# SJLeo/GCC

Measured on AMD Instinct MI355X. Metric: training images/sec at 256x256 (pix2pix GCC), higher is better.
Workload: dtype bf16

## Files before the change

gcc_amd/csrc/conv_igemm.hip:

```cpp
#include <stdlib.h>
#include <mutex>
#include "common.hpp"
#include "igemm_common.hpp"

#ifndef GCC_IGEMM_ROT
#define GCC_IGEMM_ROT 0
#endif

namespace gcc_igemm {

#ifdef GCC_CLOCK_PROBE
__device__ unsigned long long g_clock_probe[4096][8];
#endif

template <int BP, int BC, bool UT, int NS = 2, bool EV = false>
__global__ __launch_bounds__((BP / 32) * 64) void igemm_kernel(const IgemmArgs<EV> p) {
    constexpr int EPI = EV ? 1 : 0;
#include "igemm_kernel_body.inc"
}

template <int BP, int BC, bool UT, int NS = 2>
__global__ __launch_bounds__((BP / 32) * 64) void igemm_ex_kernel(const IgemmExParams p) {
    constexpr int EPI = 2;
#include "igemm_kernel_body.inc"
// ... 795 lines not shown
    auto stage_row = [&](int y) {
        char* base = ylds + ((y + 1) % 3) * row_bytes;
        const bool row_ok = (unsigned)y < (unsigned)a.Ho;
        for (int q = wave; q < pieces; q += NW) {
            const int o = q * 1024 + lane * 16;
            const int pp = o / THIN_WIDE_RB, slot = (o % THIN_WIDE_RB) >> 4;
            const int co = ((slot ^ (pp & 15)) << 3);
            const int ox = pp - 2;
            const bool ok = row_ok && (unsigned)ox < (unsigned)a.Wo && co < a.Co8;
            const uint32_t off = ok ? (uint32_t)((((n * a.Ho + y) * a.Wo + ox) * a.ldy + a.yoff + co) * 2) : OOB;
            __builtin_amdgcn_raw_ptr_buffer_load_lds(rs_y, LDS_PTR(void, base + q * 1024), 16, off, 0, 0, 0);
        }
    };
    stage_row(r_first);
    stage_row(r_first + 1);
    for (int f2 = wave; f2 < 2 * NK; f2 += NW) {
        const int py = f2 / NK, f = f2 - py * NK;
        const int u = f / (3 * NCC), b = (f / NCC) % 3 - 1, cc = f % NCC;
        const int px = i >> 3, ci = i & 7;
        const int kh = py == 0 ? (u == 0 ? 1 : 3) : (u == 0 ? 0 : 2);
        const int kw = px == 0 ? (b == 0 ? 1 : (b < 0 ? 3 : -1)) : (b > 0 ? 0 : (b == 0 ? 2 : -1));
        const int co = 32 * cc + 8 * g;
        const uint32_t off = (kw >= 0 && ci < a.Ci && co < a.Co8) ? (uint32_t)((((ci * 16 + kh * 4 + kw) * a.Co8) + co) * 2) : OOB;
        *(i32x4*)(wlds + (f2 * 64 + lane) * 16) = __builtin_amdgcn_raw_buffer_load_b128(rs_w, off, 0, 0);
    }
    int yoffs[3][NCC];
#pragma unroll
    for (int bb = 0; bb < 3; bb++)
#pragma unroll
        for (int cc = 0; cc < NCC; cc++) {
            const int pp = i + (bb - 1) + 2;
            yoffs[bb][cc] = pp * THIN_WIDE_RB + (((4 * cc + g) ^ (pp & 15)) << 4);
        }
    const int ci0 = (g & 1) * 4, pxo = g >> 1;
    float bv[4];
#pragma unroll
    for (int e = 0; e < 4; e++) bv[e] = (a.bias && ci0 + e < a.Ci) ? a.bias[ci0 + e] : 0.f;
    asm volatile("s_waitcnt vmcnt(0)" ::: "memory");
    __syncthreads();
#pragma unroll 1
    for (int r = r_first; r <= r_last; r++) {
        if (r < r_last) stage_row(r + 2);
        const char* row_u0 = ylds + ((r + 2) % 3) * row_bytes;
        const char* row_u1 = ylds + ((r + 1) % 3) * row_bytes;
#pragma unroll
        for (int pass = 0; pass < 2; pass++) {
            const int py = pass == 0 ? 1 : 0;
            const int iy = pass == 0 ? 2 * r + 1 : 2 * r + 2;
            if ((unsigned)iy >= (unsigned)a.H) continue;
            const char* wp = wlds + (py * NK * 64 + lane) * 16;
            for (int jt = wave; jt < a.tiles_per_row; jt += NW) {
                const char* t0 = row_u0 + jt * (16 * THIN_WIDE_RB);
                const char* t1 = row_u1 + jt * (16 * THIN_WIDE_RB);
                f32x4 acc0 = {0.f, 0.f, 0.f, 0.f}, acc1 = {0.f, 0.f, 0.f, 0.f};
                constexpr int PF = 4;
                bf16x8 yv[NK], wv[NK];
                auto rdy = [&](int ff) {
                    const int u = ff / (3 * NCC), bb = (ff / NCC) % 3, cc = ff % NCC;
                    return *(const bf16x8*)((u == 0 ? t0 : t1) + yoffs[bb][cc]);
                };
#pragma unroll
                for (int f = 0; f < PF; f++) { yv[f] = rdy(f); wv[f] = *(const bf16x8*)(wp + f * 1024); }
                __builtin_amdgcn_sched_group_barrier(0x100, 2 * PF, 0);
#pragma unroll
                for (int f = 0; f < NK; f++) {
                    if (f + PF < NK) { yv[f + PF] = rdy(f + PF); wv[f + PF] = *(const bf16x8*)(wp + (f + PF) * 1024); }
                    if (f & 1) acc1 = __builtin_amdgcn_mfma_f32_16x16x32_bf16(wv[f], yv[f], acc1, 0, 0, 0);
                    else acc0 = __builtin_amdgcn_mfma_f32_16x16x32_bf16(wv[f], yv[f], acc0, 0, 0, 0);
                    __builtin_amdgcn_sched_group_barrier(0x008, 1, 0);
                    if (f + PF < NK) __builtin_amdgcn_sched_group_barrier(0x100, 2, 0);
                }
                const int ix = 2 * (jt * 16 + i) + pxo;
                if (ix < a.W) {
                    float o[4];
#pragma unroll
                    for (int e = 0; e < 4; e++) {
                        o[e] = apply_act(acc0[e] + acc1[e] + bv[e], a.act, a.slope);
                        if (ci0 + e >= a.Ci) o[e] = 0.f;
                    }
                    i32x2 v = {(int)pack2bf(o[0], o[1]), (int)pack2bf(o[2], o[3])};
                    *(i32x2*)(a.dx + ((size_t)(n * a.H + iy) * a.W + ix) * a.ldx + a.xoff + ci0) = v;
                }
            }
        }
        asm volatile("s_waitcnt vmcnt(0)" ::: "memory");
        __syncthreads();
    }
}

static bool thin_dgrad_wide_shape(const gcc_conv_t* c) {
    return ceil8(c->Ci) == 8 && c->KH == 4 && c->KW == 4 && c->stride == 2 && c->pad == 1 && !(c->H & 1) && !(c->W & 1) &&
           c->Co > 64 && c->Co <= 128 && ((c->W / 2) & 3) == 0 && (size_t)(c->W / 2 + 4) * THIN_WIDE_RB * 3 + 48 * 1024 <= 156 * 1024 &&
           gcc_opt(GCC_OPT_IGEMM_THIN) >= 1 && gcc_opt(GCC_OPT_IGEMM_THIN) != 2;
}
static bool thin_dgrad_shape(const gcc_conv_t* c) {
    if (thin_dgrad_wide_shape(c)) return true;
    return ceil8(c->Ci) == 8 && c->KH == 4 && c->KW == 4 && c->stride == 2 && c->pad == 1 && !(c->H & 1) && !(c->W & 1) &&
           c->Co >= 16 && c->Co <= 64 && thin_enabled();
}
static int launch_thin_dgrad(const gcc_conv_t* c, const void* dy, const void* wt, void* dx, const gcc_epilogue_t* ep, hipStream_t st) {
    ThinDgradArgs a;
    a.dy = (const bf16_t*)dy; a.wt = (const bf16_t*)wt; a.dx = (bf16_t*)dx;
    a.bias = ep ? ep->bias : nullptr; a.act = ep ? ep->act : GCC_ACT_NONE; a.slope = ep ? ep->slope : 0.f;
    a.N = c->N; a.H = c->H; a.W = c->W; a.Ho = c->H / 2; a.Wo = c->W / 2;
    a.ldy = c->ldy; a.yoff = c->yoff; a.ldx = c->ldx; a.xoff = c->xoff; a.Ci = c->Ci; a.Co8 = ceil8(c->Co);
    const size_t yb = (size_t)c->N * a.Ho * a.Wo * c->ldy * 2, wb = (size_t)c->Ci * 16 * a.Co8 * 2;
    const size_t xb = (size_t)c->N * c->H * c->W * c->ldx * 2;
    if (yb >= OOB || wb >= OOB || xb >= OOB) return -1;
    a.dy_bytes = (uint32_t)yb; a.wt_bytes = (uint32_t)wb;
    a.tiles_per_row = cdiv(a.Wo, 16);
    a.ntiles = c->N * a.Ho * a.tiles_per_row;
    a.dTpr = make_fastdiv(a.tiles_per_row); a.dHh = make_fastdiv(a.Ho);
    if (thin_dgrad_wide_shape(c)) {
        const size_t lds = (size_t)3 * (a.Wo + 4) * THIN_WIDE_RB + 48 * 1024;
        static std::once_flag wide_once;
        std::call_once(wide_once, [] {
            (void)hipFuncSetAttribute((const void*)thin_dgrad_wide_kernel, hipFuncAttributeMaxDynamicSharedMemorySize, 156 * 1024);
        });
        int wpi = 256 / c->N;
        if (wpi < 1) wpi = 1;
        if (wpi > a.Ho) wpi = a.Ho;
        const int rows_per_wg = cdiv(a.Ho, wpi);
        wpi = cdiv(a.Ho, rows_per_wg);
        hipLaunchKernelGGL(thin_dgrad_wide_kernel, dim3(c->N * wpi), dim3(THIN_WIDE_NT), lds, st, a, rows_per_wg, wpi);
        GCC_CHECK_LAUNCH();
        return GCC_OK;
    }
    const int ncc = a.Co8 > 32 ? 2 : 1;
    int wgs = cdiv(a.ntiles, 4);
    if (wgs > 768) wgs = 768;
    const dim3 grid(wgs, 2);
    if (ncc == 2) hipLaunchKernelGGL(thin_dgrad_k4s2_kernel<2>, grid, dim3(256), 0, st, a);
    else hipLaunchKernelGGL(thin_dgrad_k4s2_kernel<1>, grid, dim3(256), 0, st, a);
    GCC_CHECK_LAUNCH();
    return GCC_OK;
}

extern "C" int gcc_conv_y2_supported(const gcc_conv_t* c, int dgrad, const gcc_epilogue_t* ep) {
    if (check_conv(c) || dgrad || !ep || !thin_shape(c)) return 0;
    if (ep->stats_partial || ep->act == GCC_ACT_TANH || (ep->act == GCC_ACT_LRELU && (ep->slope < 0.f || ep->slope > 1.f))) return 0;
    if ((ep->ldy2 & 7) || (ep->y2off & 7)) return 0;
    if (ep->y2_mode == 1) return ep->act == GCC_ACT_LRELU || ep->act == GCC_ACT_NONE;
    if (ep->y2_mode == 2) return ep->y2_gate != nullptr;
    return 0;
}

int gcc_internal_thinout_fprop(const gcc_conv_t* c, const void* x, const void* w, void* y, const gcc_epilogue_t* ep, hipStream_t st);
int gcc_internal_thinout_dgrad(const gcc_conv_t* c, const void* dy, const void* wt, void* dx, const gcc_epilogue_t* ep, hipStream_t st);
int gcc_internal_ring3(const gcc_conv_t* c, int dgrad, const void* src, const void* w, void* dst, const gcc_epilogue_t* ep, hipStream_t st);
int gcc_internal_ring3_rows(const gcc_conv_t* c, int dgrad);
bool gcc_internal_ring3_routed(const gcc_conv_t* c, int dgrad, const gcc_epilogue_t* ep);

constexpr size_t FUSE_BN_PARTIAL_BYTES = (size_t)4096 * 1024;

int gcc_internal_igemm(const gcc_conv_t* c, int dgrad, const void* src, const void* w, void* dst, const gcc_epilogue_t* ep,
                       int batch, long src_bstride, long wgt_bstride, long dst_bstride, hipStream_t st) {
    GCC_ENTER();
    int rc = check_conv(c);
    if (rc) return rc;
    if (!src || !w || !dst) return GCC_ERR_BAD_ARG;
    const int Ho = gcc_conv_out(c->H, c->KH, c->stride, c->pad);
    const int Wo = gcc_conv_out(c->W, c->KW, c->stride, c->pad);
    if (batch == 1 && head_shape(c) && ep && ep->workspace && !ep->stats_partial && (((uintptr_t)ep->workspace) & 15) == 0) {
        const int taps = c->KH * c->KW;
        if (!dgrad) {
            int ks = 1;
            const size_t need = head_fprop_workspace(c, &ks);
            if (need <= ep->workspace_bytes) {
                IgemmParams q;
                q.src = (const bf16_t*)src; q.wgt = (const bf16_t*)w; q.dst = (bf16_t*)dst; q.bias = nullptr; q.stats = nullptr;
                q.act = GCC_ACT_NONE; q.slope = 0.f;
                q.N = c->N; q.KH = 1; q.KW = 1; q.stride = 1; q.pad = 0; q.dgrad = 0;
                q.Hs = c->H; q.Ws = c->W; q.lds_ = c->ldx; q.soff = c->xoff; q.Hd = c->H; q.Wd = c->W; q.ldd = c->ldy; q.doff = c->yoff;
                q.Ct = ceil8(c->Ci); q.Cout = taps; q.ldw = q.Ct;
                const size_t rows = head_rows(c);
                const size_t sb = rows * (size_t)q.lds_ * 2, wb = (size_t)taps * q.ldw * 2;
                if (sb < OOB && wb < OOB) {
                    q.src_bytes = (uint32_t)sb; q.wgt_bytes = (uint32_t)wb;
                    q.src_bstride = q.wgt_bstride = q.dst_bstride = 0;
                    q.ntiles = 1; q.mtiles_max = cdiv((int)rows, 128);
                    const int nk = cdiv(q.Ct, BK);
                    q.ksplit = ks; q.kper = cdiv(nk, ks); q.partial = (float*)ep->workspace; q.rows_max = (int)rows; q.Cpad = 16;
                    q.raw_partial = 1;
                    int rc2 = launch<128, 16>(q, 1, 1, st);
                    if (rc2) return rc2;
                    HeadArgs a = {};
                    a.partial = q.partial; a.ksplit = q.ksplit; a.rows_max = q.rows_max; a.Cpad = 16;
                    a.bias = ep->bias; a.act = ep->act; a.slope = ep->slope;
                    a.dst = (bf16_t*)dst; a.ldd = c->ldy; a.doff = c->yoff;
                    a.N = c->N; a.H = c->H; a.W = c->W; a.Ho = Ho; a.Wo = Wo; a.KH = c->KH; a.KW = c->KW; a.stride = c->stride; a.pad = c->pad;
                    const size_t outs = (size_t)c->N * Ho * Wo;
                    hipLaunchKernelGGL(head_tapsum_kernel, dim3((unsigned)(outs + 15 > 16 * 4096 ? 4096 : (outs + 15) / 16)), dim3(256), 0, st, a);
                    GCC_CHECK_LAUNCH();
                    return GCC_OK;
                }
            }
        }
    }
    if (batch == 1 && dgrad && thin_dgrad_shape(c) && !(ep && ep->stats_partial)) {
        const int rc2 = launch_thin_dgrad(c, src, w, dst, ep, st);
        if (rc2 >= 0) return rc2;
    }
    if (batch == 1) {
        const int rc3 = dgrad ? gcc_internal_thinout_dgrad(c, src, w, dst, ep, st) : gcc_internal_thinout_fprop(c, src, w, dst, ep, st);
        if (rc3 != GCC_ERR_UNSUPPORTED) return rc3;
        const int rc4 = gcc_internal_ring3(c, dgrad, src, w, dst, ep, st);
        if (rc4 != GCC_ERR_UNSUPPORTED) return rc4;
    }
    if (ep && ep->y2) {
        if (!gcc_conv_y2_supported(c, dgrad, ep)) return GCC_ERR_UNSUPPORTED;
    }
    if (batch == 1 && !dgrad && thin_shape(c) &&
        !(ep && (ep->stats_partial || ep->act == GCC_ACT_TANH || (ep->act == GCC_ACT_LRELU && (ep->slope < 0.f || ep->slope > 1.f))))) {
        const int rc2 = launch_thin(c, src, w, dst, ep, st);
        if (rc2 >= 0) return rc2;
    }
    if (ep && ep->y2) return GCC_ERR_UNSUPPORTED;
    IgemmParams p;
    p.src = (const bf16_t*)src; p.wgt = (const bf16_t*)w; p.dst = (bf16_t*)dst;
    p.bias = ep ? ep->bias : nullptr;
    p.stats = ep ? ep->stats_partial : nullptr;
    p.act = ep ? ep->act : GCC_ACT_NONE;
    p.slope = ep ? ep->slope : 0.f;
    p.N = c->N; p.KH = c->KH; p.KW = c->KW; p.stride = c->stride; p.pad = c->pad; p.dgrad = dgrad;
    size_t src_pix, max_rows;
    if (!dgrad) {
        p.Hs = c->H; p.Ws = c->W; p.lds_ = c->ldx; p.soff = c->xoff;
        p.Hd = Ho; p.Wd = Wo; p.ldd = c->ldy; p.doff = c->yoff;
        p.Ct = ceil8(c->Ci); p.Cout = c->Co;
        max_rows = (size_t)c->N * Ho * Wo;
    } else {
        p.Hs = Ho; p.Ws = Wo; p.lds_ = c->ldy; p.soff = c->yoff;
        p.Hd = c->H; p.Wd = c->W; p.ldd = c->ldx; p.doff = c->xoff;
        p.Ct = ceil8(c->Co); p.Cout = c->Ci;
        const int s = c->stride;
        max_rows = (size_t)c->N * cdiv(c->H, s) * cdiv(c->W, s);
    }
    src_pix = (size_t)p.N * p.Hs * p.Ws;
    p.ldw = c->KH * c->KW * p.Ct;
    const size_t sb = src_pix * (size_t)p.lds_ * 2, wb = (size_t)p.Cout * p.ldw * 2;
    const size_t db = (size_t)p.N * p.Hd * p.Wd * p.ldd * 2;
    if (sb >= OOB || wb >= OOB || db >= (size_t)1 << 32) return GCC_ERR_UNSUPPORTED;
    p.src_bytes = (uint32_t)sb; p.wgt_bytes = (uint32_t)wb;
    p.src_bstride = src_bstride; p.wgt_bstride = wgt_bstride; p.dst_bstride = dst_bstride;
    if (batch < 1 || (batch > 1 && p.stats)) return GCC_ERR_BAD_ARG;
    const int phases = dgrad ? c->stride * c->stride : 1;
    if (dgrad && (c->KH < c->stride || c->KW < c->stride)) return GCC_ERR_UNSUPPORTED;
    const TilePlan tp = select_tile(c->plan, max_rows, p.Cout, phases, conv_nk(c, dgrad), batch);
    const gcc_bn_t* bnf = (ep && ep->bn && p.stats && batch == 1) ? ep->bn : nullptr;
    const int rows_alloc = p.stats ? gcc_conv_stat_tiles(c, dgrad) : 0;
    auto make_tail = [&](int rows, int wgs_per_row, TailFin* f) -> bool {
        *f = TailFin{};
        if (!bnf || !bnf->finalize_in_launch || !bnf->tail_ws || (((uintptr_t)bnf->tail_ws) & 15) || rows != rows_alloc) return false;
        if (tail_ws_bytes(rows, p.Cout) > TAIL_TICKET_BYTES + TAIL_GROUP_BYTES || bnf->tail_ws_bytes < TAIL_TICKET_BYTES + TAIL_GROUP_BYTES) return false;
        f->tickets = (unsigned*)bnf->tail_ws; f->grp = (double*)((char*)bnf->tail_ws + TAIL_TICKET_BYTES);
        f->rows = rows; f->wgs_per_row = wgs_per_row; f->count = bnf->count; f->eps = bnf->eps; f->momentum = bnf->momentum;
        f->gamma = bnf->gamma; f->beta = bnf->beta; f->running_mean = bnf->running_mean; f->running_var = bnf->running_var;
        f->mean = bnf->mean; f->rstd = bnf->rstd; f->scale = bnf->scale; f->shift = bnf->shift;
        return true;
    };
    float* const stats_rows = p.stats;
    auto finalize_after = [&]() -> int {
        if (!bnf) return GCC_OK;
        return gcc_bn_finalize(stats_rows, rows_alloc, p.Cout, bnf->count, bnf->gamma, bnf->beta, bnf->eps, bnf->momentum,
                               bnf->running_mean, bnf->running_var, bnf->mean, bnf->rstd, bnf->scale, bnf->shift, (gcc_stream_t)st);
    };
    if (batch == 1) {
        const HaloPlan h = halo_plan(c, dgrad);
        if (halo_routed(c->plan, h, dgrad, p.stats != nullptr, tp.BP)) {
            TailFin fin;
            const bool tail = p.stats && make_tail(c->N * h.tiles_x * h.tiles_y, h.ntiles, &fin);
            const int rc2 = launch_halo(c, dgrad, h, src, w, dst, ep, tail ? &fin : nullptr, st);
            if (rc2 >= 0) return (rc2 == GCC_OK && !tail) ? finalize_after() : rc2;
        }
    }
    const int BC = tp.BC;
    p.ntiles = tp.ntiles;
    p.mtiles_max = tp.mtiles;
    p.ksplit = 1; p.kper = 0; p.partial = nullptr; p.rows_max = (int)max_rows; p.Cpad = p.ntiles * BC; p.raw_partial = 0;
    p.pair = 0; p.pair_slab = nullptr; p.pair_flags = nullptr;
    p.debug = gcc_diag_bits();
    if (tp.pair && batch == 1 && ep && ep->workspace && (((uintptr_t)ep->workspace) & 15) == 0) {
        const size_t tiles = (size_t)tp.mtiles * tp.ntiles * phases;
        if (pair_workspace(tiles) <= ep->workspace_bytes) {
            p.pair = 1; p.ksplit = 2; p.kper = cdiv(conv_nk(c, dgrad), 2);
            p.pair_flags = (unsigned int*)ep->workspace;
            p.pair_slab = (float*)((char*)ep->workspace + PAIR_FLAG_BYTES);
            if (gcc_memset_async(ep->workspace, 0, PAIR_FLAG_BYTES, st) != hipSuccess) return GCC_ERR_LAUNCH;
        }
    }
    float* stats_out = p.stats;
    bool fold_stats = false;
    if (batch == 1 && tp.BP == 128 && ep && ep->workspace) {
        SplitPlan sp = plan_ksplit((long)p.mtiles_max * p.ntiles * phases, conv_nk(c, dgrad), tp.max_slices);
        if (sp.ksplit > 4 && stats_out) {
            const size_t per_slice = (size_t)phases * max_rows * p.Cpad * sizeof(float);
            const size_t cap = FUSE_BN_PARTIAL_BYTES;
            const int nk = conv_nk(c, dgrad);
            int ks = sp.ksplit;
            while (ks > 4 && per_slice * ks > cap) ks = (ks + 1) / 2;
            if (ks != sp.ksplit) { sp.kper = cdiv(nk, ks); sp.ksplit = cdiv(nk, sp.kper); }
        }
        const size_t need = (size_t)phases * sp.ksplit * max_rows * p.Cpad * sizeof(float);
        if (sp.ksplit > 1 && need <= ep->workspace_bytes && (((uintptr_t)ep->workspace) & 15) == 0) {
            p.ksplit = sp.ksplit; p.kper = sp.kper; p.partial = (float*)ep->workspace;
            p.stats = nullptr;
            fold_stats = stats_out && ceil8(p.Cout) / 8 <= 256 && rows_alloc == fold_wpp(max_rows, phases) * phases;
            if (fold_stats) p.raw_partial = 1;
        }
    }
    TailFin fin_direct;
    bool tail_direct = false;
    if (p.stats) {
        const int rows = p.mtiles_max * phases;
        if (rows != rows_alloc && gcc_memset_async(stats_out, 0, (size_t)rows_alloc * 2 * p.Cout * sizeof(float), st) != hipSuccess)
            return GCC_ERR_LAUNCH;
        tail_direct = make_tail(rows, p.ntiles, &fin_direct);
        if (tail_direct) p.fin = fin_direct;
    }
    if (tp.BP == 256) {
        rc = BC == 256 ? launch<256, 256>(p, phases, batch, st) : launch<256, 128>(p, phases, batch, st);
    } else {
        switch (BC) {
            case 128: rc = launch<128, 128>(p, phases, batch, st); break;
            case 64: rc = launch<128, 64>(p, phases, batch, st); break;
            case 32: rc = launch<128, 32>(p, phases, batch, st); break;
            default: rc = launch<128, 16>(p, phases, batch, st); break;
        }
    }
    if (rc) return rc;
    if (fold_stats) {
        FoldStatsArgs a;
        a.p = p; a.p.stats = stats_out;
        a.wpp = fold_wpp(max_rows, phases);
        a.rpw = (int)((max_rows + a.wpp - 1) / a.wpp);
        const int CH = ceil8(p.Cout) / 8;
        a.CHP = 1; a.sh = 0;
        while (a.CHP < CH) { a.CHP <<= 1; a.sh++; }
        TailFin fin;
        const bool tail = make_tail(a.wpp * phases, 1, &fin);
        a.p.fin = tail ? fin : TailFin{};
        hipLaunchKernelGGL(splitk_fold_stats_kernel, dim3(a.wpp, 1, phases), dim3(256), 0, st, a);
        GCC_CHECK_LAUNCH();
        return tail ? GCC_OK : finalize_after();
    }
    if (p.ksplit > 1 && stats_out && !p.pair) {
        const size_t pixels = (size_t)p.N * p.Hd * p.Wd;
        hipLaunchKernelGGL(channel_stats_kernel, dim3(ceil8(p.Cout) / 8), dim3(256), 0, st, p.dst, p.ldd, p.doff, p.Cout,
                           pixels, stats_out, rows_alloc);
        GCC_CHECK_LAUNCH();
        return finalize_after();
    }
    return tail_direct ? GCC_OK : finalize_after();
}

#ifdef GCC_CLOCK_PROBE
extern "C" int gcc_probe_read(unsigned long long* dst, int clear) {
    hipError_t e = hipMemcpyFromSymbol(dst, HIP_SYMBOL(gcc_igemm::g_clock_probe), sizeof(unsigned long long) * 4096 * 8);
    if (e == hipSuccess && clear) {
        void* sym = nullptr;
        if (hipGetSymbolAddress(&sym, HIP_SYMBOL(gcc_igemm::g_clock_probe)) == hipSuccess) e = hipMemset(sym, 0, sizeof(unsigned long long) * 4096 * 8);
    }
    return e == hipSuccess ? 0 : -1;
}
#endif

bool gcc_internal_thinout_routed(const gcc_conv_t* c, int dgrad, const gcc_epilogue_t* ep);
extern "C" int gcc_conv_route(const gcc_conv_t* c, int dgrad, const gcc_epilogue_t* ep) {
    if (check_conv(c)) return -1;
    if (gcc_internal_thinout_routed(c, dgrad, ep) && !(!dgrad && head_shape(c))) return 3;
    if (gcc_internal_ring3_routed(c, dgrad, ep) && !(!dgrad && head_shape(c)) && !(dgrad && thin_dgrad_shape(c) && !(ep && ep->stats_partial)))
        return 4;
    if (dgrad && thin_dgrad_shape(c) && !(ep && ep->stats_partial)) return 1;
    if (!dgrad && thin_shape(c) &&
        !(ep && (ep->stats_partial || ep->act == GCC_ACT_TANH || (ep->act == GCC_ACT_LRELU && (ep->slope < 0.f || ep->slope > 1.f)))))
        return 1;
    if (!dgrad && head_shape(c) && ep && ep->workspace && !ep->stats_partial && (((uintptr_t)ep->workspace) & 15) == 0 &&
        head_fprop_workspace(c, nullptr) <= ep->workspace_bytes)
        return 2;
    return 0;
}

namespace gcc_igemm {
struct FoldBnArgs {
    IgemmParams p;
    gcc_bn_t bn;
    int act, act2; float slope, drop_p; uint64_t seed;
    bf16_t* y; int ldy, yoff;
    bf16_t* y2; int ldy2, y2off;
    int phases;
};
template <int NT>
__global__ __launch_bounds__(NT) void splitk_bn_act_kernel(const FoldBnArgs a) {
    __shared__ double red[NT / 64][16];
    __shared__ float coef[16];
    const IgemmParams& p = a.p;
    const int c0 = blockIdx.x * 8;
    const int C = p.Cout;
    const size_t sstride = (size_t)p.rows_max * p.Cpad;
    double s[8], ss[8];
#pragma unroll
    for (int j = 0; j < 8; j++) s[j] = ss[j] = 0.0;
    for (int z = 0; z < a.phases; z++) {
        int py = 0, px = 0, Hg, Wg, ostr = 1;
        if (!p.dgrad) { Hg = p.Hd; Wg = p.Wd; }
        else {
            const int st = p.stride;
            py = z / st; px = z % st; ostr = st;
            Hg = (p.Hd - py + st - 1) / st; Wg = (p.Wd - px + st - 1) / st;
        }
        const int M = p.N * Hg * Wg;
        const float* base = p.partial + (size_t)z * p.ksplit * sstride;
        for (int m = threadIdx.x; m < M; m += NT) {
            float v[8] = {0, 0, 0, 0, 0, 0, 0, 0};
            const float* r0 = base + (size_t)m * p.Cpad + c0;
            int sl = 0;
            for (; sl + 4 <= p.ksplit; sl += 4) {
                f32x4 u[4], w[4];
#pragma unroll
                for (int q = 0; q < 4; q++) {
                    u[q] = *(const f32x4*)(r0 + (sl + q) * sstride);
                    w[q] = *(const f32x4*)(r0 + (sl + q) * sstride + 4);
                }
#pragma unroll
                for (int q = 0; q < 4; q++) {
                    v[0] += u[q][0]; v[1] += u[q][1]; v[2] += u[q][2]; v[3] += u[q][3];
                    v[4] += w[q][0]; v[5] += w[q][1]; v[6] += w[q][2]; v[7] += w[q][3];
                }
            }
            for (; sl < p.ksplit; sl++) {
                const f32x4 u = *(const f32x4*)(r0 + sl * sstride), w = *(const f32x4*)(r0 + sl * sstride + 4);
                v[0] += u[0]; v[1] += u[1]; v[2] += u[2]; v[3] += u[3];
                v[4] += w[0]; v[5] += w[1]; v[6] += w[2]; v[7] += w[3];
            }
#pragma unroll
            for (int j = 0; j < 8; j++) if (c0 + j >= C) v[j] = 0.f;
            const i32x4 pk = pack8(v);
            float r[8];
            unpack8(pk, r);
#pragma unroll
            for (int j = 0; j < 8; j++) { s[j] += (double)r[j]; ss[j] += (double)r[j] * (double)r[j]; }
            const int n = m / (Hg * Wg);
            const int rr = m - n * (Hg * Wg);
            const int oy = rr / Wg, ox = rr - oy * Wg;
            const size_t pix = (size_t)(n * p.Hd + oy * ostr + py) * p.Wd + (ox * ostr + px);
            *(i32x4*)(p.dst + pix * p.ldd + p.doff + c0) = pk;
        }
    }
    const int lane = threadIdx.x & 63, wave = threadIdx.x >> 6;
#pragma unroll
    for (int j = 0; j < 8; j++) {
#pragma unroll
        for (int o = 32; o > 0; o >>= 1) { s[j] += __shfl_xor(s[j], o, 64); ss[j] += __shfl_xor(ss[j], o, 64); }
    }
    if (lane == 0) {
#pragma unroll
        for (int j = 0; j < 8; j++) { red[wave][j] = s[j]; red[wave][8 + j] = ss[j]; }
    }
    __syncthreads();
    if (threadIdx.x < 8) {
        const int j = threadIdx.x, c = c0 + j;
        float sc = 1.f, sf = 0.f;
        if (c < C) {
            double sum = 0.0, sq = 0.0;
#pragma unroll
            for (int wv = 0; wv < NT / 64; wv++) { sum += red[wv][j]; sq += red[wv][8 + j]; }
            const double mean = sum / a.bn.count;
            double var = sq / a.bn.count - mean * mean;
            if (var < 0.0) var = 0.0;
            const float r = (float)(1.0 / sqrt(var + (double)a.bn.eps));
            const float g = a.bn.gamma ? a.bn.gamma[c] : 1.f, b = a.bn.beta ? a.bn.beta[c] : 0.f;
            if (a.bn.mean) a.bn.mean[c] = (float)mean;
            if (a.bn.rstd) a.bn.rstd[c] = r;
            sc = g * r;
            sf = b - (float)mean * g * r;
            a.bn.scale[c] = sc;
            a.bn.shift[c] = sf;
            if (a.bn.running_mean) a.bn.running_mean[c] = (1.f - a.bn.momentum) * a.bn.running_mean[c] + a.bn.momentum * (float)mean;
            if (a.bn.running_var) {
                const double unb = a.bn.count > 1.0 ? var * a.bn.count / (a.bn.count - 1.0) : var;
                a.bn.running_var[c] = (1.f - a.bn.momentum) * a.bn.running_var[c] + a.bn.momentum * (float)unb;
            }
        }
        coef[j] = sc; coef[8 + j] = sf;
    }
    __syncthreads();
    float sc[8], sf[8];
#pragma unroll
    for (int j = 0; j < 8; j++) { sc[j] = coef[j]; sf[j] = coef[8 + j]; }
    const float keep_scale = a.drop_p > 0.f ? 1.f / (1.f - a.drop_p) : 1.f;
    const size_t pixels = (size_t)p.N * p.Hd * p.Wd;
    for (int z = 0; z < a.phases; z++) {
        int py = 0, px = 0, Hg, Wg, ostr = 1;
        if (!p.dgrad) { Hg = p.Hd; Wg = p.Wd; }
        else {
            const int st = p.stride;
            py = z / st; px = z % st; ostr = st;
            Hg = (p.Hd - py + st - 1) / st; Wg = (p.Wd - px + st - 1) / st;
        }
        const int M = p.N * Hg * Wg;
        for (int m = threadIdx.x; m < M; m += NT) {
            const int n = m / (Hg * Wg);
            const int rr = m - n * (Hg * Wg);
            const int oy = rr / Wg, ox = rr - oy * Wg;
            const size_t pix = (size_t)(n * p.Hd + oy * ostr + py) * p.Wd + (ox * ostr + px);
            float v[8], o1[8], o2[8];
            unpack8(*(const i32x4*)(p.dst + pix * p.ldd + p.doff + c0), v);
#pragma unroll
            for (int j = 0; j < 8; j++) v[j] = v[j] * sc[j] + sf[j];
            if (a.drop_p > 0.f) {
#pragma unroll
                for (int j = 0; j < 8; j++) {
                    const float u = rng_uniform(a.seed, pix * (size_t)C + c0 + j);
                    v[j] = u >= a.drop_p ? v[j] * keep_scale : 0.f;
                }
            }
#pragma unroll
            for (int j = 0; j < 8; j++) if (c0 + j >= C) v[j] = 0.f;
            apply_act8(v, o1, a.act, a.slope);
            if (a.y) *(i32x4*)(a.y + pix * a.ldy + a.yoff + c0) = pack8(o1);
            if (a.y2) {
                apply_act8(v, o2, a.act2, a.slope);
                *(i32x4*)(a.y2 + pix * a.ldy2 + a.y2off + c0) = pack8(o2);
            }
        }
    }
    (void)pixels;
}
constexpr size_t FOLD_BN_MAX_ROWS = 4096;
}

static size_t al256(size_t v) { return (v + 255) & ~(size_t)255; }
extern "C" size_t gcc_conv_workspace(const gcc_conv_t* c, int dgrad);
extern "C" int gcc_conv_stat_tiles(const gcc_conv_t* c, int dgrad);
extern "C" size_t gcc_conv_bn_act_workspace(const gcc_conv_t* c, int dgrad) {
    if (check_conv(c)) return 0;
    const int Cout = dgrad ? c->Ci : c->Co;
    return al256(gcc_conv_workspace(c, dgrad)) + al256((size_t)gcc_conv_stat_tiles(c, dgrad) * 2 * Cout * sizeof(float));
}

extern "C" int gcc_conv_bn_act(const gcc_conv_t* c, int dgrad, const void* x, const void* w, void* y_raw, const gcc_bn_t* bn,
                               const gcc_bnact_t* act, void* y, int ldy, int yoff, void* y2, int ldy2, int y2off, void* ws,
                               size_t ws_bytes, gcc_stream_t stream) {
    GCC_ENTER();
    int rc = check_conv(c);
    if (rc) return rc;
    if (!x || !w || !y_raw || !bn || !act || (!y && !y2) || !bn->scale || !bn->shift || bn->count <= 0 || !ws) return GCC_ERR_BAD_ARG;
    if ((y && ((ldy & 7) || (yoff & 7))) || (y2 && ((ldy2 & 7) || (y2off & 7)))) return GCC_ERR_BAD_ARG;
    if (ws_bytes < gcc_conv_bn_act_workspace(c, dgrad) || (((uintptr_t)ws) & 15)) return GCC_ERR_WORKSPACE;
    hipStream_t st = (hipStream_t)stream;
    const int Cout = dgrad ? c->Ci : c->Co;
    const int phases = dgrad ? c->stride * c->stride : 1;
    const size_t split_bytes = al256(gcc_conv_workspace(c, dgrad));
    float* stats = (float*)((char*)ws + split_bytes);
    const int Ho = gcc_conv_out(c->H, c->KH, c->stride, c->pad), Wo = gcc_conv_out(c->W, c->KW, c->stride, c->pad);
    const size_t out_pixels = dgrad ? (size_t)c->N * c->H * c->W : (size_t)c->N * Ho * Wo;
    const int out_ld = dgrad ? c->ldx : c->ldy, out_off = dgrad ? c->xoff : c->yoff;
    const size_t max_rows = conv_max_rows(c, dgrad);
    const int nk = conv_nk(c, dgrad);
    const TilePlan tp = select_tile(c->plan, max_rows, Cout, phases, nk, 1);
    SplitPlan sp = tp.BP == 128 ? plan_ksplit((long)tp.mtiles * tp.ntiles * phases, nk, tp.max_slices) : SplitPlan{1, nk};
    if (sp.ksplit > 4 && max_rows * phases <= FOLD_BN_MAX_ROWS) {
        const size_t per_slice = (size_t)phases * max_rows * tp.ntiles * tp.BC * sizeof(float);
        const size_t cap = FUSE_BN_PARTIAL_BYTES;
        int ks = sp.ksplit;
        while (ks > 4 && per_slice * ks > cap) ks = (ks + 1) / 2;
        if (ks != sp.ksplit) { sp.kper = cdiv(nk, ks); sp.ksplit = cdiv(nk, sp.kper); }
    }
    const bool routed = (dgrad && thin_dgrad_shape(c)) || (!dgrad && thin_shape(c)) || head_shape(c);
    const int fuse = gcc_opt(GCC_OPT_FUSE_BN);
    const bool grid_ws = bn->tail_ws && bn->tail_ws_bytes >= GCC_TAIL_WORKSPACE_BYTES && (((uintptr_t)bn->tail_ws) & 15) == 0;
    if (!routed && sp.ksplit > 1 && max_rows * phases <= FOLD_BN_MAX_ROWS && (fuse == 1 || fuse == 3)) {
        FoldBnArgs a;
        IgemmParams& p = a.p;
        p.src = (const bf16_t*)x; p.wgt = (const bf16_t*)w; p.dst = (bf16_t*)y_raw; p.bias = nullptr; p.stats = nullptr;
        p.act = GCC_ACT_NONE; p.slope = 0.f;
        p.N = c->N; p.KH = c->KH; p.KW = c->KW; p.stride = c->stride; p.pad = c->pad; p.dgrad = dgrad;
        if (!dgrad) {
            p.Hs = c->H; p.Ws = c->W; p.lds_ = c->ldx; p.soff = c->xoff; p.Hd = Ho; p.Wd = Wo; p.ldd = c->ldy; p.doff = c->yoff;
            p.Ct = ceil8(c->Ci); p.Cout = c->Co;
        } else {
            p.Hs = Ho; p.Ws = Wo; p.lds_ = c->ldy; p.soff = c->yoff; p.Hd = c->H; p.Wd = c->W; p.ldd = c->ldx; p.doff = c->xoff;
            p.Ct = ceil8(c->Co); p.Cout = c->Ci;
            if (c->KH < c->stride || c->KW < c->stride) return GCC_ERR_UNSUPPORTED;
        }
        p.ldw = c->KH * c->KW * p.Ct;
        const size_t sb = (size_t)p.N * p.Hs * p.Ws * p.lds_ * 2, wb = (size_t)p.Cout * p.ldw * 2;
        if (sb >= OOB || wb >= OOB) return GCC_ERR_UNSUPPORTED;
        p.src_bytes = (uint32_t)sb; p.wgt_bytes = (uint32_t)wb;
        p.src_bstride = p.wgt_bstride = p.dst_bstride = 0;
        p.ntiles = tp.ntiles; p.mtiles_max = tp.mtiles;
        p.ksplit = sp.ksplit; p.kper = sp.kper; p.partial = (float*)ws; p.rows_max = (int)max_rows; p.Cpad = tp.ntiles * tp.BC;
        p.raw_partial = 1; p.pair = 0; p.pair_slab = nullptr; p.pair_flags = nullptr;
        if ((size_t)phases * sp.ksplit * max_rows * p.Cpad * sizeof(float) > split_bytes) return GCC_ERR_WORKSPACE;
        switch (tp.BC) {
            case 128: rc = launch<128, 128>(p, phases, 1, st); break;
            case 64: rc = launch<128, 64>(p, phases, 1, st); break;
            case 32: rc = launch<128, 32>(p, phases, 1, st); break;
            default: rc = launch<128, 16>(p, phases, 1, st); break;
        }
        if (rc) return rc;
        if (fuse == 3 && grid_ws) {
            BnFoldDesc d = {};
            d.part = p.partial; d.ksplit = p.ksplit; d.rows_max = p.rows_max; d.Cpad = p.Cpad; d.phases = phases;
            d.N = p.N; d.Hd = p.Hd; d.Wd = p.Wd; d.stride = c->stride; d.dgrad = dgrad;
            d.raw = y_raw; d.ldraw = p.ldd; d.rawoff = p.doff;
            d.y = y; d.ldy = ldy; d.yoff = yoff; d.y2 = y2; d.ldy2 = ldy2; d.y2off = y2off;
            d.C = Cout; d.bn = *bn; d.act = act->act; d.act2 = act->act2; d.slope = act->slope; d.drop_p = act->drop_p; d.seed = act->seed;
            d.ws = (char*)bn->tail_ws + TAIL_TICKET_BYTES + TAIL_GROUP_BYTES; d.ws_bytes = GCC_INORM_WORKSPACE_BYTES;
            const int rc3 = gcc_internal_bn_fold_grid(&d, st);
            if (rc3 != GCC_ERR_UNSUPPORTED) return rc3;
        }
        a.bn = *bn; a.act = act->act; a.act2 = act->act2; a.slope = act->slope; a.drop_p = act->drop_p; a.seed = act->seed;
        a.y = (bf16_t*)y; a.ldy = ldy; a.yoff = yoff; a.y2 = (bf16_t*)y2; a.ldy2 = ldy2; a.y2off = y2off; a.phases = phases;
        hipLaunchKernelGGL(splitk_bn_act_kernel<1024>, dim3(ceil8(Cout) / 8), dim3(1024), 0, st, a);
        GCC_CHECK_LAUNCH();
        return GCC_OK;
    }
    gcc_bn_t bnf = *bn;
    if (!gcc_opt(GCC_OPT_FUSE_BN)) { bnf.tail_ws = nullptr; bnf.tail_ws_bytes = 0; }
    gcc_epilogue_t ep = {nullptr, GCC_ACT_NONE, 0.f, stats, split_bytes ? ws : nullptr, split_bytes, &bnf, nullptr, 0, 0, 0, nullptr};
    rc = gcc_internal_igemm(c, dgrad, x, w, y_raw, &ep, 1, 0, 0, 0, st);
    if (rc) return rc;
    gcc_bnact_t q = *act;
    q.scale = bn->scale; q.shift = bn->shift; q.gate = nullptr; q.gate_after_act = 0; q.groups = 1; q.residual = nullptr; q.ld_residual = 0;
    return gcc_bnact_fwd(&q, y_raw, out_ld, out_off, y, ldy, yoff, y2, ldy2, y2off, Cout, out_pixels, stream);
}

extern "C" size_t gcc_conv_workspace(const gcc_conv_t* c, int dgrad) {
    if (check_conv(c)) return 0;
    if (head_shape(c) && !dgrad) return head_fprop_workspace(c, nullptr);
    const int phases = dgrad ? c->stride * c->stride : 1;
    const size_t max_rows = conv_max_rows(c, dgrad);
    const int nk = conv_nk(c, dgrad);
    const TilePlan tp = select_tile(c->plan, max_rows, dgrad ? c->Ci : c->Co, phases, nk, 1);
    if (tp.pair) return pair_workspace((size_t)tp.mtiles * tp.ntiles * phases);
    if (tp.BP != 128) return 0;
    const SplitPlan sp = plan_ksplit((long)tp.mtiles * tp.ntiles * phases, nk, tp.max_slices);
    if (sp.ksplit <= 1) return 0;
    return (size_t)phases * sp.ksplit * max_rows * tp.ntiles * tp.BC * sizeof(float);
}

extern "C" int gcc_conv_tile(const gcc_conv_t* c, int dgrad) {
    if (check_conv(c)) return 0;
    const int phases = dgrad ? c->stride * c->stride : 1;
    const TilePlan tp = select_tile(c->plan, conv_max_rows(c, dgrad), dgrad ? c->Ci : c->Co, phases, conv_nk(c, dgrad), 1);
    return tp.BP * 1000 + tp.BC;
}

extern "C" int gcc_conv_stat_tiles(const gcc_conv_t* c, int dgrad) {
    GCC_ENTER();
    if (check_conv(c)) return 0;
    if (const int r3 = gcc_internal_ring3_rows(c, dgrad)) return r3;
    const int phases = dgrad ? c->stride * c->stride : 1;
    const TilePlan tp = select_tile(c->plan, conv_max_rows(c, dgrad), dgrad ? c->Ci : c->Co, phases, conv_nk(c, dgrad), 1);
    const HaloPlan h = halo_plan(c, dgrad);
    if (halo_routed(c->plan, h, dgrad, true, tp.BP)) return c->N * h.tiles_x * h.tiles_y;
    if (tp.BP == 128 && ceil8(dgrad ? c->Ci : c->Co) / 8 <= 256) {
        const SplitPlan sp = plan_ksplit((long)tp.mtiles * tp.ntiles * phases, conv_nk(c, dgrad), tp.max_slices);
        if (sp.ksplit > 1) return fold_wpp(conv_max_rows(c, dgrad), phases) * phases;
    }
    return tp.mtiles * phases;
}

extern "C" int gcc_conv_fprop(const gcc_conv_t* c, const void* x, const void* w, void* y,
                              const gcc_epilogue_t* ep, gcc_stream_t stream) {
    GCC_ENTER();
    return gcc_internal_igemm(c, 0, x, w, y, ep, 1, 0, 0, 0, (hipStream_t)stream);
}

extern "C" int gcc_conv_dgrad(const gcc_conv_t* c, const void* dy, const void* wt, void* dx,
                              const gcc_epilogue_t* ep, gcc_stream_t stream) {
    GCC_ENTER();
    return gcc_internal_igemm(c, 1, dy, wt, dx, ep, 1, 0, 0, 0, (hipStream_t)stream);
}

int gcc_internal_ring3_eval(const gcc_conv_t* c, const void* src, const void* w, void* dst, const EvalEpi& ev, hipStream_t st);
bool gcc_internal_ring3_eval_routed(const gcc_conv_t* c);

namespace {
TilePlan eval_tile(const gcc_conv_t* c) {
    gcc_conv_plan_t pl = c->plan;
    pl.tile_families = 1;
    return select_tile(pl, conv_max_rows(c, 0), c->Co, 1, conv_nk(c, 0), 1);
}
SplitPlan eval_split_plan(const gcc_conv_t* c, const TilePlan& tp) {
    return plan_ksplit((long)tp.mtiles * tp.ntiles, conv_nk(c, 0), tp.max_slices);
}
size_t eval_split_bytes(const gcc_conv_t* c, const TilePlan& tp) {
    const SplitPlan sp = eval_split_plan(c, tp);
    return sp.ksplit > 1 ? (size_t)sp.ksplit * conv_max_rows(c, 0) * tp.ntiles * tp.BC * sizeof(float) : 0;
}
SplitPlan eval_split(const gcc_conv_t* c, const TilePlan& tp, const void* ws, size_t ws_bytes) {
    const SplitPlan none = {1, conv_nk(c, 0)};
    const size_t need = eval_split_bytes(c, tp);
    if (!need || !ws || (((uintptr_t)ws) & 15) || need > ws_bytes) return none;
    return eval_split_plan(c, tp);
}

int igemm_eval(const gcc_conv_t* c, const void* x, const void* w, void* y, const EvalEpi& ev, void* ws, size_t ws_bytes,
               hipStream_t st) {
    const int Ho = gcc_conv_out(c->H, c->KH, c->stride, c->pad), Wo = gcc_conv_out(c->W, c->KW, c->stride, c->pad);
    IgemmEvParams p;
    p.src = (const bf16_t*)x; p.wgt = (const bf16_t*)w; p.dst = (bf16_t*)y;
    p.bias = nullptr; p.stats = nullptr; p.act = GCC_ACT_NONE; p.slope = 0.f;
    p.N = c->N; p.KH = c->KH; p.KW = c->KW; p.stride = c->stride; p.pad = c->pad; p.dgrad = 0;
    p.Hs = c->H; p.Ws = c->W; p.lds_ = c->ldx; p.soff = c->xoff;
    p.Hd = Ho; p.Wd = Wo; p.ldd = c->ldy; p.doff = c->yoff;
    p.Ct = ceil8(c->Ci); p.Cout = c->Co;
    p.ldw = c->KH * c->KW * p.Ct;
    const size_t max_rows = (size_t)c->N * Ho * Wo;
    const size_t sb = (size_t)c->N * c->H * c->W * (size_t)p.lds_ * 2, wb = (size_t)p.Cout * p.ldw * 2;
    const size_t db = max_rows * p.ldd * 2;
    if (sb >= OOB || wb >= OOB || db >= (size_t)1 << 32 || max_rows >= (size_t)1 << 31) return GCC_ERR_UNSUPPORTED;
    p.src_bytes = (uint32_t)sb; p.wgt_bytes = (uint32_t)wb;
    p.src_bstride = p.wgt_bstride = p.dst_bstride = 0;
    const TilePlan tp = eval_tile(c);
    if (tp.BP != 128) return GCC_ERR_UNSUPPORTED;
    p.ntiles = tp.ntiles; p.mtiles_max = tp.mtiles;
    const SplitPlan sp = eval_split(c, tp, ws, ws_bytes);
    p.ksplit = sp.ksplit; p.kper = sp.kper; p.partial = sp.ksplit > 1 ? (float*)ws : nullptr;
    p.rows_max = (int)max_rows; p.Cpad = tp.ntiles * tp.BC; p.raw_partial = 0;
    p.pair = 0; p.pair_slab = nullptr; p.pair_flags = nullptr;
    p.debug = 0;
    p.ev = ev;
    switch (tp.BC) {
        case 128: return launch_eval<128>(p, st);
        case 64: return launch_eval<64>(p, st);
        case 32: return launch_eval<32>(p, st);
        default: return launch_eval<16>(p, st);
    }
}
}

extern "C" size_t gcc_conv_eval_workspace(const gcc_conv_t* c) {
    if (check_conv(c) || gcc_internal_ring3_eval_routed(c)) return 0;
    return eval_split_bytes(c, eval_tile(c));
}

extern "C" int gcc_conv_eval_route(const gcc_conv_t* c, size_t workspace_bytes) {
    if (check_conv(c)) return -1;
    if (gcc_internal_ring3_eval_routed(c)) return 4;
    const size_t need = eval_split_bytes(c, eval_tile(c));
    return need && need <= workspace_bytes ? 5 : 0;
}

extern "C" int gcc_conv_fprop_eval(const gcc_conv_t* c, const void* x, const void* w, void* y, const gcc_eval_epilogue_t* ep,
                                   gcc_stream_t stream) {
    GCC_ENTER();
    int rc = check_conv(c);
    if (rc) return rc;
    if (!x || !w || !y || !ep) return GCC_ERR_BAD_ARG;
    if (ep->act < GCC_EVAL_ACT_NONE || ep->act > GCC_EVAL_ACT_TANH || (ep->act == GCC_EVAL_ACT_PRELU && !ep->slope)) return GCC_ERR_BAD_ARG;
    if (ep->residual && ((ep->ld_residual & 7) || (ep->residual_off & 7) || ep->ld_residual < ep->residual_off + ceil8(c->Co)))
        return GCC_ERR_BAD_ARG;
    EvalEpi ev;
    ev.scale = ep->scale; ev.shift = ep->shift; ev.slope = ep->slope; ev.res = (const bf16_t*)ep->residual;
    ev.ldr = ep->ld_residual; ev.roff = ep->residual_off; ev.act = ep->act;
    const hipStream_t st = (hipStream_t)stream;
    rc = gcc_internal_ring3_eval(c, x, w, y, ev, st);
    if (rc != GCC_ERR_UNSUPPORTED) return rc;
    return igemm_eval(c, x, w, y, ev, ep->workspace, ep->workspace_bytes, st);
}

namespace {
TilePlan ex_tile(const gcc_conv_t* c, int dg) {
    gcc_conv_plan_t pl = c->plan;
    pl.tile_families = 1;
    return select_tile(pl, conv_max_rows(c, dg), dg ? c->Ci : c->Co, dg ? c->stride * c->stride : 1, conv_nk(c, dg), 1);
}
SplitPlan ex_split_plan(const gcc_conv_t* c, int dg, const TilePlan& tp) {
    const int phases = dg ? c->stride * c->stride : 1;
    return plan_ksplit((long)tp.mtiles * tp.ntiles * phases, conv_nk(c, dg), tp.max_slices);
}
size_t ex_split_bytes(const gcc_conv_t* c, int dg, const TilePlan& tp) {
    const SplitPlan sp = ex_split_plan(c, dg, tp);
    const size_t phases = dg ? (size_t)c->stride * c->stride : 1;
    return sp.ksplit > 1 ? phases * sp.ksplit * conv_max_rows(c, dg) * tp.ntiles * tp.BC * sizeof(float) : 0;
}
int ex_geometry(const gcc_conv_t* c, int dg) {
    if (dg && (c->KH < c->stride || c->KW < c->stride)) return GCC_ERR_UNSUPPORTED;
    const int Ho = gcc_conv_out(c->H, c->KH, c->stride, c->pad), Wo = gcc_conv_out(c->W, c->KW, c->stride, c->pad);
    const size_t xpix = (size_t)c->N * c->H * c->W, ypix = (size_t)c->N * Ho * Wo;
    const size_t sb = (dg ? ypix * c->ldy : xpix * c->ldx) * 2, db = (dg ? xpix * c->ldx : ypix * c->ldy) * 2;
    const size_t wb = (size_t)(dg ? c->Ci : c->Co) * c->KH * c->KW * ceil8(dg ? c->Co : c->Ci) * 2;
    if (sb >= OOB || wb >= OOB || db >= (size_t)1 << 32 || conv_max_rows(c, dg) >= (size_t)1 << 31) return GCC_ERR_UNSUPPORTED;
    return GCC_OK;
}
bool ex_act_ok(int a) {
    return a == GCC_EVAL_ACT_NONE || a == GCC_EVAL_ACT_RELU || a == GCC_EVAL_ACT_LRELU || a == GCC_EVAL_ACT_TANH;
}
}

// ... 85 lines not shown
```

Baseline: 1089.

## Add register-resident split-K kernel for small-map 4x4 stride-2 convolutions

Adds a dedicated MFMA kernel for 4x4 stride-2 pad-1 convs with tiny output maps (up to 64 rows). Each wave keeps a K-slice of weights in registers and streams the few output pixels, writing fp32 partials that the existing split-K epilogue or BN fold reduces. The goal is to replace the 128-row tile igemm, which mostly pads and idles on the deep U-Net bottleneck layers, with a K-sliced grid that fills the GPU. The workspace sizing is widened to cover the extra slices, and the new plan may raise partial-buffer traffic.

```diff
diff --git a/gcc_amd/csrc/conv_igemm.hip b/gcc_amd/csrc/conv_igemm.hip
--- a/gcc_amd/csrc/conv_igemm.hip
+++ b/gcc_amd/csrc/conv_igemm.hip
@@ -971,6 +971,28 @@
 bool gcc_internal_ring3_routed(const gcc_conv_t* c, int dgrad, const gcc_epilogue_t* ep);
 
 constexpr size_t FUSE_BN_PARTIAL_BYTES = (size_t)4096 * 1024;
+
+namespace gcc_igemm {
+int smallmap_blocks(const gcc_conv_t* c, int dgrad, size_t max_rows, int Cpad, int phases, int nk, size_t cap);
+int launch_smallmap(const IgemmParams& p, int phases, hipStream_t st);
+}
+static bool smallmap_split(const gcc_conv_t* c, int dgrad, const TilePlan& tp, size_t max_rows, int phases, int nk, SplitPlan* sp) {
+    if (tp.BP != 128 || sp->ksplit < 2) return false;
+    const int kb = smallmap_blocks(c, dgrad, max_rows, tp.ntiles * tp.BC, phases, nk, FUSE_BN_PARTIAL_BYTES);
+    if (!kb) return false;
+    sp->kper = kb; sp->ksplit = cdiv(nk, kb);
+    return true;
+}
+static int launch_small(const IgemmParams& p, int phases, hipStream_t st) {
+    const int rc = launch_smallmap(p, phases, st);
+    if (rc || p.raw_partial) return rc;
+    const size_t total = (size_t)p.rows_max * (ceil8(p.Cout) / 8);
+    int blocks = (int)((total + 255) / 256);
+    if (blocks > 1024) blocks = 1024;
+    hipLaunchKernelGGL(splitk_epilogue_kernel<false>, dim3(blocks, 1, phases), dim3(256), 0, st, p);
+    GCC_CHECK_LAUNCH();
+    return GCC_OK;
+}
 
 int gcc_internal_igemm(const gcc_conv_t* c, int dgrad, const void* src, const void* w, void* dst, const gcc_epilogue_t* ep,
                        int batch, long src_bstride, long wgt_bstride, long dst_bstride, hipStream_t st) {
@@ -1110,6 +1132,7 @@
     }
     float* stats_out = p.stats;
     bool fold_stats = false;
+    bool small = false;
     if (batch == 1 && tp.BP == 128 && ep && ep->workspace) {
         SplitPlan sp = plan_ksplit((long)p.mtiles_max * p.ntiles * phases, conv_nk(c, dgrad), tp.max_slices);
         if (sp.ksplit > 4 && stats_out) {
@@ -1120,6 +1143,7 @@
             while (ks > 4 && per_slice * ks > cap) ks = (ks + 1) / 2;
             if (ks != sp.ksplit) { sp.kper = cdiv(nk, ks); sp.ksplit = cdiv(nk, sp.kper); }
         }
+        small = smallmap_split(c, dgrad, tp, max_rows, phases, conv_nk(c, dgrad), &sp);
         const size_t need = (size_t)phases * sp.ksplit * max_rows * p.Cpad * sizeof(float);
         if (sp.ksplit > 1 && need <= ep->workspace_bytes && (((uintptr_t)ep->workspace) & 15) == 0) {
             p.ksplit = sp.ksplit; p.kper = sp.kper; p.partial = (float*)ep->workspace;
@@ -1137,7 +1161,9 @@
         tail_direct = make_tail(rows, p.ntiles, &fin_direct);
         if (tail_direct) p.fin = fin_direct;
     }
-    if (tp.BP == 256) {
+    if (small && p.ksplit > 1) {
+        rc = launch_small(p, phases, st);
+    } else if (tp.BP == 256) {
         rc = BC == 256 ? launch<256, 256>(p, phases, batch, st) : launch<256, 128>(p, phases, batch, st);
     } else {
         switch (BC) {
@@ -1386,6 +1412,7 @@
         while (ks > 4 && per_slice * ks > cap) ks = (ks + 1) / 2;
         if (ks != sp.ksplit) { sp.kper = cdiv(nk, ks); sp.ksplit = cdiv(nk, sp.kper); }
     }
+    const bool small = smallmap_split(c, dgrad, tp, max_rows, phases, nk, &sp);
     const bool routed = (dgrad && thin_dgrad_shape(c)) || (!dgrad && thin_shape(c)) || head_shape(c);
     const int fuse = gcc_opt(GCC_OPT_FUSE_BN);
     const bool grid_ws = bn->tail_ws && bn->tail_ws_bytes >= GCC_TAIL_WORKSPACE_BYTES && (((uintptr_t)bn->tail_ws) & 15) == 0;
@@ -1412,7 +1439,8 @@
         p.ksplit = sp.ksplit; p.kper = sp.kper; p.partial = (float*)ws; p.rows_max = (int)max_rows; p.Cpad = tp.ntiles * tp.BC;
         p.raw_partial = 1; p.pair = 0; p.pair_slab = nullptr; p.pair_flags = nullptr;
         if ((size_t)phases * sp.ksplit * max_rows * p.Cpad * sizeof(float) > split_bytes) return GCC_ERR_WORKSPACE;
-        switch (tp.BC) {
+        if (small) rc = launch_small(p, phases, st);
+        else switch (tp.BC) {
             case 128: rc = launch<128, 128>(p, phases, 1, st); break;
             case 64: rc = launch<128, 64>(p, phases, 1, st); break;
             case 32: rc = launch<128, 32>(p, phases, 1, st); break;
@@ -1457,7 +1485,9 @@
     if (tp.BP != 128) return 0;
     const SplitPlan sp = plan_ksplit((long)tp.mtiles * tp.ntiles * phases, nk, tp.max_slices);
     if (sp.ksplit <= 1) return 0;
-    return (size_t)phases * sp.ksplit * max_rows * tp.ntiles * tp.BC * sizeof(float);
+    SplitPlan sm = sp;
+    const int slices = smallmap_split(c, dgrad, tp, max_rows, phases, nk, &sm) && sm.ksplit > sp.ksplit ? sm.ksplit : sp.ksplit;
+    return (size_t)phases * slices * max_rows * tp.ntiles * tp.BC * sizeof(float);
 }
 
 extern "C" int gcc_conv_tile(const gcc_conv_t* c, int dgrad) {
diff --git a/gcc_amd/csrc/conv_smallmap.hip b/gcc_amd/csrc/conv_smallmap.hip
--- /dev/null
+++ b/gcc_amd/csrc/conv_smallmap.hip
@@ -0,0 +1,129 @@
+#include "common.hpp"
+#include "igemm_common.hpp"
+
+namespace gcc_igemm {
+
+constexpr size_t SMALLMAP_MAX_ROWS = 64;
+constexpr size_t SMALLMAP_MAX_L2_BYTES = (size_t)16 << 20;
+constexpr int SMALLMAP_MAX_SLICES = 16;
+constexpr int SMALLMAP_MAX_KB = 16;
+constexpr long SMALLMAP_FILL_WAVES = 1024;
+
+constexpr int SM_K = 4, SM_S = 2, SM_PAD = 1;
+
+__device__ __forceinline__ int floor_div12(int a, int s) { return s == 2 ? (a >> 1) : a; }
+__device__ __forceinline__ int dgrad_tap_row(int tap, int dgrad) { return dgrad ? tap >> 1 : tap >> 2; }
+
+template <int KB>
+__global__ __launch_bounds__(256) void smallmap_kernel(const IgemmParams p) {
+    const int lane = threadIdx.x & 63;
+    const int wave = __builtin_amdgcn_readfirstlane(threadIdx.x >> 6);
+    const int lr = lane & 15, lq = lane >> 4;
+    const int co0 = (blockIdx.x * 4 + wave) * 16;
+    if (co0 >= p.Cpad || co0 >= ceil8(p.Cout)) return;
+
+    int Hg, Wg, sy, TB, dy0, dx0, dstep, kh0, kw0, kstep, nk_all;
+    if (!p.dgrad) {
+        Hg = p.Hd; Wg = p.Wd; sy = SM_S; TB = SM_K;
+        dy0 = -SM_PAD; dx0 = -SM_PAD; dstep = 1; kh0 = 0; kw0 = 0; kstep = 1;
+        nk_all = (SM_K * SM_K * p.Ct) / BK;
+    } else {
+        const int py = blockIdx.z / SM_S, px = blockIdx.z % SM_S;
+        kh0 = (py + SM_PAD) % SM_S; kw0 = (px + SM_PAD) % SM_S;
+        TB = SM_K / SM_S;
+        dy0 = (py + SM_PAD - kh0) / SM_S; dx0 = (px + SM_PAD - kw0) / SM_S;
+        dstep = -1; kstep = SM_S; sy = 1;
+        Hg = (p.Hd - py + SM_S - 1) / SM_S; Wg = (p.Wd - px + SM_S - 1) / SM_S;
+        nk_all = ((SM_K / SM_S) * (SM_K / SM_S) * p.Ct) / BK;
+    }
+    const int M = p.N * Hg * Wg;
+    const int sl = blockIdx.y;
+    const __amdgpu_buffer_rsrc_t rs_src = __builtin_amdgcn_make_buffer_rsrc((void*)p.src, 0, p.src_bytes, 0x00020000);
+    const __amdgpu_buffer_rsrc_t rs_wgt = __builtin_amdgcn_make_buffer_rsrc((void*)p.wgt, 0, p.wgt_bytes, 0x00020000);
+
+    int b_dy[KB], b_dx[KB], b_pix[KB];
+    bool b_ok[KB];
+    bf16x8 w[KB][2];
+    const int wrow = co0 + lr;
+    const int wbase = wrow * p.ldw * 2 + lq * 32;
+    const bool wok = wrow < p.Cout;
+    int tap = (sl * KB * BK) / p.Ct;
+    int cc = sl * KB * BK - tap * p.Ct;
+    int ta = dgrad_tap_row(tap, p.dgrad), tb = tap - ta * TB;
+#pragma unroll
+    for (int b = 0; b < KB; b++) {
+        b_dy[b] = dy0 + ta * dstep; b_dx[b] = dx0 + tb * dstep;
+        b_pix[b] = ((ta * p.Ws + tb) * dstep * p.lds_ + cc) * 2;
+        const int oy_lo = max(0, -floor_div12(b_dy[b], sy)), oy_hi = min(Hg - 1, floor_div12(p.Hs - 1 - b_dy[b], sy));
+        const int ox_lo = max(0, -floor_div12(b_dx[b], sy)), ox_hi = min(Wg - 1, floor_div12(p.Ws - 1 - b_dx[b], sy));
+        b_ok[b] = (sl * KB + b < nk_all) & (oy_lo <= oy_hi) & (ox_lo <= ox_hi);
+        const int wt_off = (((kh0 + ta * kstep) * SM_K + (kw0 + tb * kstep)) * p.Ct + cc) * 2;
+        const uint32_t off = (b_ok[b] & wok) ? (uint32_t)(wbase + wt_off) : OOB;
+        w[b][0] = __builtin_bit_cast(bf16x8, __builtin_amdgcn_raw_buffer_load_b128(rs_wgt, off, 0, 0));
+        w[b][1] = __builtin_bit_cast(bf16x8, __builtin_amdgcn_raw_buffer_load_b128(rs_wgt, off + 16, 0, 0));
+        cc += BK;
+        if (cc == p.Ct) { cc = 0; if (++tb == TB) { tb = 0; ++ta; } }
+    }
+
+    float* part = p.partial + ((size_t)(blockIdx.z * p.ksplit + sl) * p.rows_max) * p.Cpad + co0 + 4 * lq;
+    const int HW = Hg * Wg;
+    for (int m0 = 0; m0 < M; m0 += 16) {
+        const int m = m0 + lr;
+        const bool mv = m < M;
+        const int n = m / HW;
+        const int r = m - n * HW;
+        const int oy = r / Wg, ox = r - oy * Wg;
+        const int iy0 = oy * sy, ix0 = ox * sy;
+        const int base = (((n * p.Hs + iy0 + dy0) * p.Ws + ix0 + dx0) * p.lds_ + p.soff) * 2 + lq * 32;
+        bf16x8 x[KB][2];
+#pragma unroll
+        for (int b = 0; b < KB; b++) {
+            const bool ok = mv & b_ok[b] & ((unsigned)(iy0 + b_dy[b]) < (unsigned)p.Hs) & ((unsigned)(ix0 + b_dx[b]) < (unsigned)p.Ws);
+            const uint32_t off = ok ? (uint32_t)(base + b_pix[b]) : OOB;
+            x[b][0] = __builtin_bit_cast(bf16x8, __builtin_amdgcn_raw_buffer_load_b128(rs_src, off, 0, 0));
+            x[b][1] = __builtin_bit_cast(bf16x8, __builtin_amdgcn_raw_buffer_load_b128(rs_src, off + 16, 0, 0));
+        }
+        f32x4 acc = {0.f, 0.f, 0.f, 0.f};
+#pragma unroll
+        for (int b = 0; b < KB; b++) {
+            acc = __builtin_amdgcn_mfma_f32_16x16x32_bf16(w[b][0], x[b][0], acc, 0, 0, 0);
+            acc = __builtin_amdgcn_mfma_f32_16x16x32_bf16(w[b][1], x[b][1], acc, 0, 0, 0);
+        }
+        __builtin_amdgcn_sched_group_barrier(0x020, 2 * KB, 0);
+        __builtin_amdgcn_sched_group_barrier(0x008, 2 * KB, 0);
+        if (mv) *(f32x4*)(part + (size_t)m * p.Cpad) = acc;
+    }
+}
+
+int smallmap_blocks(const gcc_conv_t* c, int dgrad, size_t max_rows, int Cpad, int phases, int nk, size_t cap) {
+    if (c->KH != 4 || c->KW != 4 || c->stride != 2 || c->pad != 1) return 0;
+    const int Ct = ceil8(dgrad ? c->Co : c->Ci);
+    if ((Ct % BK) || max_rows > SMALLMAP_MAX_ROWS || (Cpad & 15) || nk < 2) return 0;
+    if ((size_t)phases * nk * max_rows * (BK * 2) * (Cpad / 16) > SMALLMAP_MAX_L2_BYTES) return 0;
+    int KB = 1;
+    while (KB < SMALLMAP_MAX_KB && cdiv(nk, KB) > SMALLMAP_MAX_SLICES) KB *= 2;
+    if (cdiv(nk, KB) > SMALLMAP_MAX_SLICES) return 0;
+    auto waves = [&](int kb) { return (long)phases * (Cpad / 16) * cdiv(nk, kb); };
+    auto bytes = [&](int kb) { return (size_t)phases * cdiv(nk, kb) * max_rows * Cpad * sizeof(float); };
+    while (KB < SMALLMAP_MAX_KB && cdiv(nk, 2 * KB) >= 2 && waves(2 * KB) >= SMALLMAP_FILL_WAVES) KB *= 2;
+    while (KB < SMALLMAP_MAX_KB && cdiv(nk, 2 * KB) >= 2 && bytes(KB) > cap) KB *= 2;
+    if (bytes(KB) > cap) return 0;
+    return KB;
+}
+
+int launch_smallmap(const IgemmParams& p, int phases, hipStream_t st) {
+    if (!p.partial || p.ksplit < 2 || (p.Cpad & 15) || (p.Ct % BK)) return GCC_ERR_BAD_ARG;
+    const dim3 grid(cdiv(p.Cpad / 16, 4), p.ksplit, phases), block(256);
+    switch (p.kper) {
+        case 1: hipLaunchKernelGGL(smallmap_kernel<1>, grid, block, 0, st, p); break;
+        case 2: hipLaunchKernelGGL(smallmap_kernel<2>, grid, block, 0, st, p); break;
+        case 4: hipLaunchKernelGGL(smallmap_kernel<4>, grid, block, 0, st, p); break;
+        case 8: hipLaunchKernelGGL(smallmap_kernel<8>, grid, block, 0, st, p); break;
+        case 16: hipLaunchKernelGGL(smallmap_kernel<16>, grid, block, 0, st, p); break;
+        default: return GCC_ERR_BAD_ARG;
+    }
+    GCC_CHECK_LAUNCH();
+    return GCC_OK;
+}
+
+}
```

Result: no change. 1087 (-0.1%).
